# NorthStarUAS/ImageAnalysis

Measured on AMD Instinct MI355X. Metric: image_pairs_matched_per_sec, higher is better.
Workload: dtype u8 (int8 MFMA, int32 accumulate)

## Files before the change

imageanalysis_amd/csrc/match_knn2sym.hip:

```cpp
#include "iamx_common.h"
#include "sym_cand_rule.h"

namespace {

typedef int v4i __attribute__((ext_vector_type(4)));
typedef int v2i __attribute__((ext_vector_type(2)));
typedef int v16i __attribute__((ext_vector_type(16)));
typedef unsigned v2u __attribute__((ext_vector_type(2)));

#ifndef IAMX_DESC_OFFSET
#define IAMX_DESC_OFFSET 128
#endif
constexpr int D = IAMX_DESC_DIM;
constexpr int CHUNK = 128;
constexpr int BIG = 0x3F000000;

struct Pack3Args {
    const void *src;
    const int64_t *src_off;
    int64_t single_n;
    const int32_t *dst_off;
    int8_t *dst;
    int32_t *sn2, *sct, *sperm, *sinv;
    int32_t *n2, *nb, *pos;
// ... 183 lines not shown
            P.sn2[d0 + r] = 0;
            P.sct[d0 + r] = BIG;
            P.sperm[d0 + r] = -1;
            P.sinv[d0 + r] = -1;
        }
        return;
    }
    const SRC *p = static_cast<const SRC *>(P.src) + (r0 + r) * D + part * 16;
    unsigned w[4] = {0, 0, 0, 0};
#pragma unroll
    for (int i = 0; i < 16; ++i)
        w[i >> 2] |= (unsigned)((load_value(p, i) - IAMX_DESC_OFFSET) & 0xFF) << (8 * (i & 3));
    const int pos = d0 + P.pos[r0 + r];
    *reinterpret_cast<uint4 *>(P.dst + (int64_t)pos * D + part * 16) = make_uint4(w[0], w[1], w[2], w[3]);
    if (part == 0) {
        P.sn2[pos] = P.n2[r0 + r];
        P.sct[pos] = P.nb[r0 + r] >> 1;
        P.sperm[pos] = r;
        P.sinv[d0 + r] = pos - d0;
    }
}

constexpr int ROW_NO_BOUND = 0x7F000000;
__device__ __forceinline__ int pack_row_bounds(int L, int U1, int U2)
{
#if defined(IAMX_T_NOPACK)
    return U1;
#else
    typedef unsigned short us2 __attribute__((ext_vector_type(2)));
    const us2 d = __builtin_amdgcn_cvt_pk_u16((unsigned)(U1 - L), (unsigned)(U2 - L));
    return (int)__builtin_bit_cast(unsigned, d);
#endif
}
__device__ __forceinline__ void unpack_row_bounds(v2i e, int &L, int &U1, int &U2)
{
    const int d1 = e.y & 0xFFFF, d2 = (int)((unsigned)e.y >> 16);
    L = e.x;
    U1 = d1 == 0xFFFF ? ROW_NO_BOUND : e.x + d1;
    U2 = d2 == 0xFFFF ? ROW_NO_BOUND : e.x + d2;
}

struct SymArgs {
    const int8_t *sdesc;
    const int32_t *sn2, *sct;
    const int32_t *img_off, *img_n;
    const int32_t *upairs;
    const int32_t *wg_off;
    const int64_t *col_off;
    const int64_t *rowp_off;
    int32_t *col;
    int32_t *rowp;
    int n_u, total_wg;
    uint8_t *colmask;
};

__device__ __forceinline__ int uniform32(int x) { return __builtin_amdgcn_readfirstlane(x); }
__device__ __forceinline__ int64_t uniform64(int64_t x)
{
    return (int64_t)(((uint64_t)(unsigned)__builtin_amdgcn_readfirstlane((int)(x >> 32)) << 32) |
                     (unsigned)__builtin_amdgcn_readfirstlane((int)x));
}

template <bool FUSED>
__device__ __forceinline__ void half_wave_min16(int (&r)[16], int lo, int &m0, int &m1)
{
    int u[4], w[2];
    if constexpr (FUSED) {
        asm("s_nop 1\n\t"
            "v_min_i32_dpp %0, %0, %0 row_ror:8 row_mask:0xf bank_mask:0x3\n\t"
            "v_min_i32_dpp %0, %8, %8 row_ror:8 row_mask:0xf bank_mask:0xc\n\t"
            "v_min_i32_dpp %1, %1, %1 row_ror:8 row_mask:0xf bank_mask:0x3\n\t"
            "v_min_i32_dpp %1, %9, %9 row_ror:8 row_mask:0xf bank_mask:0xc\n\t"
            "v_min_i32_dpp %2, %2, %2 row_ror:8 row_mask:0xf bank_mask:0x3\n\t"
            "v_min_i32_dpp %2, %10, %10 row_ror:8 row_mask:0xf bank_mask:0xc\n\t"
            "v_min_i32_dpp %3, %3, %3 row_ror:8 row_mask:0xf bank_mask:0x3\n\t"
            "v_min_i32_dpp %3, %11, %11 row_ror:8 row_mask:0xf bank_mask:0xc\n\t"
            "v_min_i32_dpp %4, %4, %4 row_ror:8 row_mask:0xf bank_mask:0x3\n\t"
            "v_min_i32_dpp %4, %12, %12 row_ror:8 row_mask:0xf bank_mask:0xc\n\t"
            "v_min_i32_dpp %5, %5, %5 row_ror:8 row_mask:0xf bank_mask:0x3\n\t"
            "v_min_i32_dpp %5, %13, %13 row_ror:8 row_mask:0xf bank_mask:0xc\n\t"
            "v_min_i32_dpp %6, %6, %6 row_ror:8 row_mask:0xf bank_mask:0x3\n\t"
            "v_min_i32_dpp %6, %14, %14 row_ror:8 row_mask:0xf bank_mask:0xc\n\t"
            "v_min_i32_dpp %7, %7, %7 row_ror:8 row_mask:0xf bank_mask:0x3\n\t"
            "v_min_i32_dpp %7, %15, %15 row_ror:8 row_mask:0xf bank_mask:0xc"
            : "+v"(r[0]), "+v"(r[2]), "+v"(r[4]), "+v"(r[6]), "+v"(r[8]), "+v"(r[10]), "+v"(r[12]), "+v"(r[14])
            : "v"(r[1]), "v"(r[3]), "v"(r[5]), "v"(r[7]), "v"(r[9]), "v"(r[11]), "v"(r[13]), "v"(r[15]));
        asm("s_nop 1\n\t"
            "v_min_i32_dpp %0, %0, %0 row_ror:12 row_mask:0xf bank_mask:0x5\n\t"
            "v_min_i32_dpp %0, %4, %4 row_ror:4 row_mask:0xf bank_mask:0xa\n\t"
            "v_min_i32_dpp %1, %1, %1 row_ror:12 row_mask:0xf bank_mask:0x5\n\t"
            "v_min_i32_dpp %1, %5, %5 row_ror:4 row_mask:0xf bank_mask:0xa\n\t"
            "v_min_i32_dpp %2, %2, %2 row_ror:12 row_mask:0xf bank_mask:0x5\n\t"
            "v_min_i32_dpp %2, %6, %6 row_ror:4 row_mask:0xf bank_mask:0xa\n\t"
            "v_min_i32_dpp %3, %3, %3 row_ror:12 row_mask:0xf bank_mask:0x5\n\t"
            "v_min_i32_dpp %3, %7, %7 row_ror:4 row_mask:0xf bank_mask:0xa"
            : "+v"(r[0]), "+v"(r[4]), "+v"(r[8]), "+v"(r[12])
            : "v"(r[2]), "v"(r[6]), "v"(r[10]), "v"(r[14]));
#pragma unroll
        for (int k = 0; k < 4; ++k) u[k] = r[4 * k] + lo;
    } else {
        int s[8];
#pragma unroll
        for (int k = 0; k < 8; ++k) {
            const int a = r[2 * k], b = r[2 * k + 1];
            const int t1 = __builtin_amdgcn_update_dpp(b, a, 0x128, 0xF, 0x3, false);
            const int t2 = __builtin_amdgcn_update_dpp(a, b, 0x128, 0xF, 0xC, false);
// ... 55 lines not shown
            "v_min_i32_dpp %1, %1, %1 row_ror:12 row_mask:0xf bank_mask:0x5\n\t"
            "v_min_i32_dpp %1, %5, %5 row_ror:4 row_mask:0xf bank_mask:0xa\n\t"
            "v_min_i32_dpp %2, %2, %2 row_ror:12 row_mask:0xf bank_mask:0x5\n\t"
            "v_min_i32_dpp %2, %6, %6 row_ror:4 row_mask:0xf bank_mask:0xa\n\t"
            "v_min_i32_dpp %3, %3, %3 row_ror:12 row_mask:0xf bank_mask:0x5\n\t"
            "v_min_i32_dpp %3, %7, %7 row_ror:4 row_mask:0xf bank_mask:0xa"
            : "+v"(r[0]), "+v"(r[4]), "+v"(r[8]), "+v"(r[12])
            : "v"(r[2]), "v"(r[6]), "v"(r[10]), "v"(r[14]));
#pragma unroll
        for (int k = 0; k < 4; ++k) u[k] = r[4 * k] + lo;
    } else {
        int w[2];
#pragma unroll
        for (int k = 0; k < 2; ++k) {
            const v2u x = __builtin_amdgcn_permlane16_swap((unsigned)u[2 * k], (unsigned)u[2 * k + 1], false, false);
            w[k] = min((int)x[0], (int)x[1]);
        }
#pragma unroll
        for (int k = 0; k < 2; ++k) {
            w[k] = min(w[k], __builtin_amdgcn_update_dpp(0, w[k], 0xB1, 0xF, 0xF, true));
            w[k] = min(w[k], __builtin_amdgcn_update_dpp(0, w[k], 0x4E, 0xF, 0xF, true));
        }
        dst[0] = w[0];
        dst[16] = w[1];
    }
}

template <int P, bool PASS>
__device__ __forceinline__ void row_min16_block(int (&r)[16], int &after)
{
    static_assert(P >= 0 && P < 6, "six blocks");
    int keep = after;
    if constexpr (P < 4) {
        asm("s_nop 1\n\t"
            "v_min_i32_dpp %0, %0, %0 row_ror:8 row_mask:0xf bank_mask:0x3\n\t"
            "v_min_i32_dpp %0, %3, %3 row_ror:8 row_mask:0xf bank_mask:0xc\n\t"
            "v_min_i32_dpp %1, %1, %1 row_ror:8 row_mask:0xf bank_mask:0x3\n\t"
            "v_min_i32_dpp %1, %4, %4 row_ror:8 row_mask:0xf bank_mask:0xc"
            : "+v"(r[4 * P]), "+v"(r[4 * P + 2]), "+v"(keep)
            : "v"(r[4 * P + 1]), "v"(r[4 * P + 3]));
    } else {
        constexpr int Q = 8 * (P - 4);
        asm("s_nop 1\n\t"
            "v_min_i32_dpp %0, %0, %0 row_ror:12 row_mask:0xf bank_mask:0x5\n\t"
            "v_min_i32_dpp %0, %3, %3 row_ror:4 row_mask:0xf bank_mask:0xa\n\t"
            "v_min_i32_dpp %1, %1, %1 row_ror:12 row_mask:0xf bank_mask:0x5\n\t"
            "v_min_i32_dpp %1, %4, %4 row_ror:4 row_mask:0xf bank_mask:0xa"
            : "+v"(r[Q]), "+v"(r[Q + 4]), "+v"(keep)
            : "v"(r[Q + 2]), "v"(r[Q + 6]));
    }
    if constexpr (PASS) after = keep;
}

constexpr int sweep_gap_valu(int nv, int tail, bool blocks, int g)
{
    const int last = tail < 6 ? 6 - tail : 0;
    const int rest = nv - last - (blocks ? 2 : 0), n = blocks ? 5 : 7;
    if (g == 7) return last;
    if (blocks && (g == 3 || g == 4)) return 1;
    const int i = blocks && g > 4 ? g - 2 : g;
    return rest / n + (i < rest % n ? 1 : 0);
}

template <int V> struct int_c { static constexpr int value = V; };
template <int FROM, int TO, typename F>
__device__ __forceinline__ void static_for(F &&f)
{
    if constexpr (FROM < TO) {
        f(int_c<FROM>{});
        static_for<FROM + 1, TO>(f);
    }
}

template <int QW, int NW, int VARIANT, int PIPE, int MERGEW, int SLEEP, bool GROUPLO, int CH, int WPE>
__global__ __launch_bounds__(NW * 64, WPE) void knn2sym_kernel(SymArgs A)
{
    static_assert((VARIANT == 0 || VARIANT == 1) && PIPE > 0 && MERGEW == 2 && SLEEP == 0 && GROUPLO && CH == 128,
                  "only the shipped sweep is implemented");
    constexpr bool ITEMS = VARIANT == 1;
    constexpr int CHUNK = CH;
    constexpr int WGROWS = NW * QW * 32;
    constexpr int NT = NW * 64;
    constexpr int PIECES = CHUNK * D / 16 / NT;
    __shared__ __attribute__((aligned(16))) int8_t lds[2 * CHUNK * D + 2 * CHUNK * 4 + 3 * NW * CHUNK * 4 + 2 * NW * 4 + (2 * NW * CHUNK + NW * 256) * 4];
    int8_t *lds_tile = lds;
    int *lds_tb = reinterpret_cast<int *>(lds + 2 * CHUNK * D);
    int *lds_row = lds_tb + 2 * CHUNK;
    int *lds_cq = lds_row + 3 * NW * CHUNK;
    int *lds_dump = lds_cq + 2 * NW;
    const int tid = threadIdx.x, lane = tid & 63, wave = tid >> 6;
    const int c = lane & 31, g = lane >> 5;

    int vid;
    {
        const int total = A.total_wg, bid = blockIdx.x;
        const int xcd = bid & 7, k = bid >> 3, q = total >> 3, r = total & 7;
        vid = (xcd < r ? xcd * (q + 1) : r * (q + 1) + (xcd - r) * q) + k;
    }
    int lo = 0, hi = A.n_u;
    if constexpr (!ITEMS)
        while (hi - lo > 1) {
            const int mid = (lo + hi) >> 1;
            if (A.wg_off[mid] <= vid) lo = mid; else hi = mid;
        }
    int u = lo, u_end = 0, item_wgi = 0;
    if constexpr (ITEMS) {
        u = A.wg_off[3 * vid];
        u_end = u + A.wg_off[3 * vid + 1];
        item_wgi = A.wg_off[3 * vid + 2];
    }
    v4i bq[QW][4];
    int lo_lane;
    int bimg_held = -1;
    if constexpr (ITEMS) asm volatile("" : "+v"(u_end), "+v"(item_wgi), "+v"(bimg_held));
    int nx_b = 0, nx_a = 0, nx_boff = 0, nx_nb = 0, nx_aoff = 0, nx_na = 0;
    int64_t nx_rowp = 0;
    if constexpr (ITEMS) {
        nx_b = A.upairs[2 * u];
        nx_a = A.upairs[2 * u + 1];
        nx_boff = A.img_off[nx_b];
        nx_nb = A.img_n[nx_b];
        nx_aoff = A.img_off[nx_a];
        nx_na = A.img_n[nx_a];
        nx_rowp = A.rowp_off[u];
    }
    for (;;) {
        const int bimg = ITEMS ? uniform32(nx_b) : A.upairs[2 * u], aimg = ITEMS ? uniform32(nx_a) : A.upairs[2 * u + 1];
        const int boff = ITEMS ? uniform32(nx_boff) : A.img_off[bimg], nb = ITEMS ? uniform32(nx_nb) : A.img_n[bimg];
        const int aoff = ITEMS ? uniform32(nx_aoff) : A.img_off[aimg], na = ITEMS ? uniform32(nx_na) : A.img_n[aimg];
        const int capA = (na + CHUNK - 1) / CHUNK * CHUNK;
        const int nchunks = capA / CHUNK;
        const int wgi = ITEMS ? uniform32(item_wgi) : vid - A.wg_off[u];
        const int q0 = wgi * WGROWS + wave * (QW * 32);
        const bool wave_valid = q0 < nb;
        const int64_t rbase = (ITEMS ? uniform64(nx_rowp) : A.rowp_off[u]) + (int64_t)wgi * capA;
        if constexpr (ITEMS)
            if (uniform32(bimg_held) >= 0) __syncthreads();

        const int rc = (c & 16) | ((c & 3) << 2) | ((c >> 2) & 3);
        if (!ITEMS || bimg != uniform32(bimg_held)) {
            bimg_held = bimg;
#pragma unroll
            for (int qb = 0; qb < QW; ++qb) {
                int row = q0 + QW * rc + qb;
                row = row < nb ? row : nb - 1;
                const v4i *src = reinterpret_cast<const v4i *>(A.sdesc + (int64_t)(boff + row) * D);
#pragma unroll
                for (int s = 0; s < 4; ++s) {
                    bq[qb][s] = ~src[2 * s + g];
                    if constexpr (WPE == 1) asm volatile("" : "+a"(bq[qb][s]));
                }
            }
            lo_lane = 0;
            {
                int spread = 0;
                if (wave_valid) {
                    const int g_lo = rc & ~3, g_hi = rc | 3;
                    const int r_lo = q0 + QW * g_lo < nb ? q0 + QW * g_lo : nb - 1;
                    const int r_hi = q0 + QW * g_hi + QW - 1 < nb ? q0 + QW * g_hi + QW - 1 : nb - 1;
                    lo_lane = A.sn2[boff + r_lo] >> 1;
                    spread = (A.sn2[boff + r_hi] >> 1) - lo_lane;
                }
#pragma unroll
                for (int sh = 32; sh >= 1; sh >>= 1) spread = max(spread, __shfl_xor(spread, sh));
                if (lane == 0) lds_cq[wave] = spread;
            }
        }
// ... 14 lines not shown
        auto stage_direct = [&](int ch, int buf) {
#pragma unroll
            for (int j = 0; j < PIECES; ++j) {
                const int e = j * NT + tid, row = e >> 3, slot = (e & 7) ^ ((row >> 1) & 7);
                const int8_t *gsrc = tbase + (int64_t)(ch * CHUNK + row) * D + slot * 16;
                int8_t *ldst = lds_tile + buf * (CHUNK * D) + (j * NT + wave * 64) * 16;
                __builtin_amdgcn_global_load_lds(gsrc, (lds_ptr)ldst, 16, 0, 0);
            }
            __builtin_amdgcn_global_load_lds(tci + ch * CHUNK + (tid & (CHUNK - 1)),
                                             (lds_ptr)(lds_tb + buf * CHUNK + (wave & (CHUNK / 64 - 1)) * 64), 4, 0, 0);
        };
        auto wait_direct = [&]() { __builtin_amdgcn_s_waitcnt(0x0F70); };
        constexpr int MROWS = CHUNK / MERGEW;
        static_assert(MROWS == 64 && NW % MERGEW == 0, "one merge row per lane");
        const int mrow = (wave % MERGEW) * MROWS + lane;
        const bool merger = wave < MERGEW;
        constexpr int RSRC_WORD3_DATA_FORMAT_32 = 4 << 15;
        constexpr int RANGE_DROP = 0x7FFFFFF0;
        const __amdgpu_buffer_rsrc_t rowp_rsrc =
            __builtin_amdgcn_make_buffer_rsrc(A.rowp + 2 * rbase, (short)0, capA * 8, RSRC_WORD3_DATA_FORMAT_32);
        int spread_w[NW];
        auto merge_rows = [&](int ch, int rbo, bool store) {
            int L = BIG, U1 = BIG, U2 = BIG;
#pragma unroll
            for (int w = 0; w < NW; ++w) {
                const int R = lds_row[rbo + w * CHUNK + mrow];
                const int lw = R, uw = R + spread_w[w];
                L = min(L, lw);
                U2 = min(max(U1, uw), U2);
                U1 = min(U1, uw);
            }
            __builtin_amdgcn_raw_buffer_store_b64(v2i{L, pack_row_bounds(L, U1, U2)}, rowp_rsrc,
                                                  store ? (ch * CHUNK + mrow) * 8 : RANGE_DROP, 0, 0);
        };

        constexpr int PP = QW / 2, NT4 = CHUNK / 32, NS = NT4 * PP;
        static_assert(NT4 % 2 == 0 && NT4 >= 2, "tile parity must carry across chunks");
        int *const row_dst = (lane & 3) == 0 && wave_valid
            ? lds_row + wave * CHUNK + 8 * ((lane >> 4) & 1) + 4 * g + 2 * ((lane >> 2) & 1) + ((lane >> 3) & 1)
            : lds_dump + wave * 256 + lane;
        v4i aop[2][4], tbop[2][4];
        v16i accs[2][2];
        int r[2][16], bu[4];
#pragma unroll
        for (int k = 0; k < 16; ++k) r[1][k] = BIG;
        auto load_op = [&](int buf, int tile, int k, v4i (&a)[4], v4i (&tbv)[4]) {
            if (k < 4) {
                tbv[k] = *reinterpret_cast<const v4i *>(lds_tb + buf * CHUNK + tile * 32 + 8 * k + 4 * g);
            } else {
                const int s = k - 4, rr = tile * 32 + c, swz = (rr >> 1) & 7;
                a[s] = *reinterpret_cast<const v4i *>(lds_tile + buf * (CHUNK * D) + rr * D + (((2 * s + g) ^ swz) * 16));
            }
        };
        auto issue = [&](int t, int qp, v16i &acc0, v16i &acc1) {
#pragma unroll
            for (int reg = 0; reg < 16; ++reg) acc0[reg] = acc1[reg] = tbop[t & 1][reg >> 2][reg & 3];
#pragma unroll
            for (int s = 0; s < 4; ++s) {
                acc0 = __builtin_amdgcn_mfma_i32_32x32x32_i8(aop[t & 1][s], bq[qp][s], acc0, 0, 0, 0);
                acc1 = __builtin_amdgcn_mfma_i32_32x32x32_i8(aop[t & 1][s], bq[qp + 1][s], acc1, 0, 0, 0);
            }
            if constexpr (WPE == 1) asm volatile("" : "+v"(acc0), "+v"(acc1));
        };

        if constexpr (ITEMS) {
            const int un = u + 1 < u_end ? u + 1 : u;
            nx_b = A.upairs[2 * un];
            nx_a = A.upairs[2 * un + 1];
            nx_rowp = A.rowp_off[un];
        }
        stage_direct(0, 0);
        stage_direct(nchunks > 1 ? 1 : 0, 1);
        wait_direct();
        __syncthreads();
#pragma unroll
        for (int w = 0; w < NW; ++w) spread_w[w] = __builtin_amdgcn_readfirstlane(lds_cq[w]);
        if constexpr (ITEMS) {
            const int b = uniform32(nx_b), a = uniform32(nx_a);
            nx_boff = A.img_off[b];
            nx_nb = A.img_n[b];
            nx_aoff = A.img_off[a];
            nx_na = A.img_n[a];
        }
#pragma unroll
        for (int k = 0; k < 8; ++k) load_op(0, 0, k, aop[0], tbop[0]);
#pragma unroll
        for (int k = 0; k < 8 / PP; ++k) load_op(0, 1, k, aop[1], tbop[1]);
        issue(0, 0, accs[0][0], accs[0][1]);
        __builtin_amdgcn_sched_barrier(0);
        int rbo = 0, rbo_prev = 2 * NW * CHUNK;
        const int wave_u = uniform32(wave);
        typedef __attribute__((address_space(3))) const int8_t *lds_bytes;
        int opoff[4], tboff = 2 * CHUNK * D + 16 * g;
#pragma unroll
        for (int s = 0; s < 4; ++s) opoff[s] = c * D + (((2 * s + g) ^ ((c >> 1) & 7)) * 16);
        auto load_op_at = [&](int tile, int k, v4i (&a)[4], v4i (&tbv)[4]) {
            if (k < 4) tbv[k] = *reinterpret_cast<const __attribute__((address_space(3))) v4i *>((lds_bytes)lds + tboff + tile * 128 + 32 * k);
            else a[k - 4] = *reinterpret_cast<const __attribute__((address_space(3))) v4i *>((lds_bytes)lds + opoff[k - 4] + tile * (32 * D));
        };
        const unsigned stage_voff = (unsigned)((tid >> 3) * D + (((tid & 7) ^ ((tid >> 4) & 7)) * 16));
        const unsigned ct_voff = (unsigned)((tid & (CHUNK - 1)) * 4);
        for (int ch = 0; ch < nchunks; ++ch) {
            const int buf = ch & 1;
            if constexpr (PP == 4) {
            constexpr int BAR = (NT4 - 1) * PP - 1;
            static_assert(NW == 4 && PIECES == 4 && BAR + 4 < NS && (NT / 8) % 16 == 0, "the gaps below are form 2's");
            const int chs = ch + 2 < nchunks ? ch + 2 : nchunks - 1;
            const int8_t *const sg_tile = tbase + (int64_t)chs * (CHUNK * D);
            const int8_t *const sg_ct = reinterpret_cast<const int8_t *>(tci + chs * CHUNK);
            int mR[NW], mL = BIG, mU1 = BIG, mU2 = BIG;
            static_for<0, NS>([&](auto st_c) {
                constexpr int st = decltype(st_c)::value;
                constexpr int t = st / PP, ph = st % PP, qp = 2 * ph, cur = st & 1;
                constexpr int nst = st + 1 < NS ? st + 1 : 0;
                if constexpr (st == BAR) {
                    __builtin_amdgcn_s_waitcnt(0x0070);
                    __syncthreads();
                }
                issue(nst / PP, 2 * (nst % PP), accs[cur ^ 1][0], accs[cur ^ 1][1]);
                static_for<(st == BAR - 1 ? 1 : 0), (st == BAR - 2 ? 2 : 1)>([&](auto d_c) {
                    constexpr int sr = st + decltype(d_c)::value;
                    constexpr int T = (sr + 1) / PP + 1, i = (sr + 1) % PP;
                    if constexpr (T == NT4 && i == 0) {
#pragma unroll
                        for (int s = 0; s < 4; ++s) opoff[s] ^= CHUNK * D;
                        tboff ^= CHUNK * 4;
                    }
#pragma unroll
                    for (int k = i * 8 / PP; k < (i + 1) * 8 / PP; ++k) load_op_at(T % NT4, k, aop[T & 1], tbop[T & 1]);
                });
                constexpr int nv = (ph == 2 ? 36 : ph == 3 ? 40 : 32) + (st == BAR + 2 ? 11 : 0) + (st == BAR + 3 ? 5 : 0) +
                                   (st >= BAR && st <= BAR + PIECES ? 1 : 0) +
                                   (st == NS - 1 ? 2 : 0);
                constexpr int tail = (st == BAR - 1 ? 0 : st == BAR - 2 ? 4 : 2) + (ph == 3 ? 1 + 2 : 0) + (st >= BAR && st <= BAR + PIECES ? 1 : 0) +
                                     (st == BAR + 1 ? 2 : 0) + (st == BAR + 3 ? 1 : 0);
                constexpr int blk_at = sweep_gap_valu(nv, tail, true, 0) + sweep_gap_valu(nv, tail, true, 1) +
                                       sweep_gap_valu(nv, tail, true, 2) - 16;
                static_assert(ph == 3 || (blk_at >= 0 && blk_at < 15 && blk_at != 7), "gaps 3 and 4 hold two minima of one column chain");
                const v16i acc0 = accs[cur][0], acc1 = accs[cur][1];
                int (&rc_)[16] = r[t & 1];
                int (&rp)[16] = r[(t + 1) & 1];
#pragma unroll
                for (int reg = 0; reg < 16; ++reg)
                    rc_[reg] = qp == 0 ? min(acc0[reg], acc1[reg]) : min(min(rc_[reg], acc0[reg]), acc1[reg]);
                static_for<0, 16>([&](auto w_c) {
                    constexpr int w = decltype(w_c)::value;
                    int &mm = m[qp + (w >> 3)][t & 3];
                    const v16i &acc = w < 8 ? acc0 : acc1;
                    mm = min(min(mm, acc[2 * (w & 7)]), acc[2 * (w & 7) + 1]);
                    if constexpr (ph < 3 && w == blk_at) row_min16_block<2 * ph, true>(rp, mm);
                    if constexpr (ph < 3 && w == blk_at + 1) row_min16_block<2 * ph + 1, true>(rp, mm);
                });
                if constexpr (ph == 2) {
#pragma unroll
                    for (int k = 0; k < 4; ++k) bu[k] = rp[4 * k] + lo_lane;
                }
                if constexpr (ph == 3) {
                    int *const dst = row_dst + (t > 0 ? rbo : rbo_prev) + (t > 0 ? t - 1 : NT4 - 1) * 32;
                    row_min16_piece<3>(rp, bu, lo_lane, dst);
                }
                if constexpr (st >= BAR && st < BAR + PIECES)
                    __builtin_amdgcn_global_load_lds(sg_tile + (st - BAR) * ((NT / 8) * D) + stage_voff,
                                                     (lds_ptr)(lds_tile + buf * (CHUNK * D) + ((st - BAR) * NT + wave_u * 64) * 16), 16, 0, 0);
                if constexpr (st == BAR + PIECES)
                    __builtin_amdgcn_global_load_lds(sg_ct + ct_voff,
                                                     (lds_ptr)(lds_tb + buf * CHUNK + (wave_u & (CHUNK / 64 - 1)) * 64), 4, 0, 0);
                if constexpr (st == BAR + 1) {
#pragma unroll
                    for (int w = 0; w < NW; ++w) mR[w] = lds_row[rbo_prev + w * CHUNK + mrow];
                }
                if constexpr (st == BAR + 2) {
#pragma unroll
                    for (int w = 0; w < NW; ++w) {
                        const int uw = mR[w] + spread_w[w];
                        mL = min(mL, mR[w]);
                        mU2 = min(max(mU1, uw), mU2);
                        mU1 = min(mU1, uw);
                    }
                }
                if constexpr (st == BAR + 3)
                    __builtin_amdgcn_raw_buffer_store_b64(v2i{mL, pack_row_bounds(mL, mU1, mU2)}, rowp_rsrc,
                                                          merger && ch > 0 ? ((ch - 1) * CHUNK + mrow) * 8 : RANGE_DROP, 0, 0);
                static_for<0, 8>([&](auto g_c) {
                    constexpr int g = decltype(g_c)::value;
                    __builtin_amdgcn_sched_group_barrier(0x008, 1, 0);
                    __builtin_amdgcn_sched_group_barrier(0x002, sweep_gap_valu(nv, tail, ph < 3, g) + (g == 7 ? 3 : 0), 0);
                });
                __builtin_amdgcn_sched_barrier(0);
            });
            } else {
#pragma unroll
            for (int st = 0; st < NS; ++st) {
                const int t = st / PP, qp = 2 * (st % PP), cur = st & 1;
                if (st == (NT4 - 1) * PP - 1) {
                    __builtin_amdgcn_s_waitcnt(0x0070);
                    __syncthreads();
                    stage_direct(ch + 2 < nchunks ? ch + 2 : nchunks - 1, buf);
                    merge_rows(ch - 1, rbo_prev, merger && ch > 0);
                }
                if (st + 1 < NS) issue((st + 1) / PP, 2 * ((st + 1) % PP), accs[cur ^ 1][0], accs[cur ^ 1][1]);
                else issue(0, 0, accs[cur ^ 1][0], accs[cur ^ 1][1]);
                {
                    const int T = (st + 1) / PP + 1, i = (st + 1) % PP;
#pragma unroll
                    for (int k = i * 8 / PP; k < (i + 1) * 8 / PP; ++k)
                        load_op(T < NT4 ? buf : buf ^ 1, T % NT4, k, aop[T & 1], tbop[T & 1]);
                }
                const v16i acc0 = accs[cur][0], acc1 = accs[cur][1];
                int t0 = min(min(m[qp][t & 3], acc0[0]), acc0[1]);
                int t1m = min(min(m[qp + 1][t & 3], acc1[0]), acc1[1]);
#pragma unroll
                for (int reg = 2; reg < 16; reg += 2) {
                    t0 = min(min(t0, acc0[reg]), acc0[reg + 1]);
                    t1m = min(min(t1m, acc1[reg]), acc1[reg + 1]);
                }
                m[qp][t & 3] = t0;
                m[qp + 1][t & 3] = t1m;
                int (&rc_)[16] = r[t & 1];
                if (qp == 0) {
#pragma unroll
                    for (int reg = 0; reg < 16; ++reg) rc_[reg] = min(acc0[reg], acc1[reg]);
                } else {
#pragma unroll
                    for (int reg = 0; reg < 16; ++reg) rc_[reg] = min(min(rc_[reg], acc0[reg]), acc1[reg]);
                }
                {
                    int (&rp)[16] = r[(t + 1) & 1];
                    const int tp = t > 0 ? t - 1 : NT4 - 1;
                    int *dst = row_dst + (t > 0 ? rbo : rbo_prev) + tp * 32;
                    if constexpr (PP == 1) {
                        int m0, m1;
                        half_wave_min16<true>(rp, lo_lane, m0, m1);
                        dst[0] = m0;
                        dst[16] = m1;
                    } else {
                        if (0 * PP / 4 == st % PP) row_min16_piece<0>(rp, bu, lo_lane, dst);
                        if (1 * PP / 4 == st % PP) row_min16_piece<1>(rp, bu, lo_lane, dst);
                        if (2 * PP / 4 == st % PP) row_min16_piece<2>(rp, bu, lo_lane, dst);
                        if (3 * PP / 4 == st % PP) row_min16_piece<3>(rp, bu, lo_lane, dst);
                    }
                }
#pragma unroll
                for (int i = 0; i < 8; ++i) {
                    __builtin_amdgcn_sched_group_barrier(0x008, 1, 0);
                    __builtin_amdgcn_sched_group_barrier(0x002, PIPE, 0);
                }
                __builtin_amdgcn_sched_barrier(0);
            }
            }
            rbo_prev = rbo;
            rbo = rbo == 2 * NW * CHUNK ? 0 : rbo + NW * CHUNK;
        }
        int64_t col_v = 0;
        if constexpr (ITEMS) col_v = A.col_off[u];
        {
            int m0, m1;
            half_wave_min16<true>(r[(NT4 - 1) & 1], lo_lane, m0, m1);
            int *dst = row_dst + rbo_prev + (NT4 - 1) * 32;
            dst[0] = m0;
            dst[16] = m1;
        }
        wait_direct();
        __syncthreads();
        merge_rows(nchunks - 1, rbo_prev, merger);

        const int64_t col_u = ITEMS ? uniform64(col_v) : 0;
        if (wave_valid) {
            unsigned ownpack = 0;
            int v1s[QW], v2s[QW];
#pragma unroll
            for (int qb = 0; qb < QW; ++qb) {
                const int lo01 = min(m[qb][0], m[qb][1]), hi01 = max(m[qb][0], m[qb][1]);
                const int lo23 = min(m[qb][2], m[qb][3]), hi23 = max(m[qb][2], m[qb][3]);
                const int a1 = min(lo01, lo23), a2 = min(max(lo01, lo23), min(hi01, hi23));
                const int b1 = __shfl_xor(a1, 32), b2 = __shfl_xor(a2, 32);
                const int v1 = min(a1, b1), v2 = min(max(a1, b1), min(a2, b2));
                v1s[qb] = v1;
                v2s[qb] = v2;
#if !defined(IAMX_T_NOMASK)
                const unsigned own = (m[qb][0] <= v2 ? 1u : 0u) | (m[qb][1] <= v2 ? 2u : 0u) |
                                     (m[qb][2] <= v2 ? 4u : 0u) | (m[qb][3] <= v2 ? 8u : 0u);
                ownpack |= own << (4 * qb);
#endif
            }
            const unsigned othpack = A.colmask ? (unsigned)__shfl_xor((int)ownpack, 32) : 0u;
            const int row0 = q0 + QW * rc;
            if (g == 0) {
#pragma unroll
                for (int qb = 0; qb < QW; ++qb)
                    if (row0 + qb < nb)
                        *reinterpret_cast<v2i *>(A.col + 2 * ((ITEMS ? col_u : A.col_off[u]) + row0 + qb)) = v2i{v1s[qb], v2s[qb]};
                if (A.colmask) {
                    uint8_t *dst = A.colmask + (ITEMS ? col_u : A.col_off[u]) + row0;
                    if (QW == 8 && row0 + QW <= nb) {
                        auto spread = [](unsigned nib4) {
                            const unsigned x = (nib4 | (nib4 << 8)) & 0x00FF00FFu;
                            return (x | (x << 4)) & 0x0F0F0F0Fu;
                        };
                        const unsigned lo = spread(ownpack & 0xFFFFu) | (spread(othpack & 0xFFFFu) << 4);
                        const unsigned hi = spread(ownpack >> 16) | (spread(othpack >> 16) << 4);
                        *reinterpret_cast<v2u *>(dst) = v2u{lo, hi};
                    } else {
#pragma unroll
                        for (int qb = 0; qb < QW; ++qb)
                            if (row0 + qb < nb)
// ... 1055 lines not shown
                       dim3((unsigned)(((int64_t)cap * 8 + 255) / 256), (unsigned)P.n_img),
                       dim3(256), 0, st, P);
    return iamx::check_launch(what);
}

template <typename SRC>
static int pack3_single(const SRC *src, int64_t n_rows, int8_t *dst, int32_t *sn2, int32_t *sct,
                        int32_t *sperm, int32_t *sinv, int32_t *scratch, void *stream,
                        const char *what)
{
    if (n_rows < 0 || n_rows > (1 << 24) || (n_rows > 0 && !src) || !dst || !sn2 || !sct || !sperm ||
        !sinv || !scratch)
        return iamx::fail(IAMX_EINVAL, "%s: null pointer or bad row count", what);
    Pack3Args P{src, nullptr, n_rows, nullptr, dst, sn2, sct, sperm, sinv,
                scratch, scratch + n_rows, scratch + 2 * n_rows, 1};
    return pack3_launch<SRC>(P, n_rows, (int)n_rows, stream, what);
}

extern "C" int iamx_desc3_pack_u8(const uint8_t *src, int64_t n_rows, int8_t *dst, int32_t *sn2,
                                  int32_t *sct, int32_t *sperm, int32_t *sinv, int32_t *scratch,
                                  void *stream)
{
    return pack3_single(src, n_rows, dst, sn2, sct, sperm, sinv, scratch, stream, "iamx_desc3_pack_u8");
}

extern "C" int iamx_desc3_pack_f32(const float *src, int64_t n_rows, int8_t *dst, int32_t *sn2,
                                   int32_t *sct, int32_t *sperm, int32_t *sinv, int32_t *scratch,
                                   void *stream)
{
    return pack3_single(src, n_rows, dst, sn2, sct, sperm, sinv, scratch, stream, "iamx_desc3_pack_f32");
}

extern "C" int iamx_desc3_pack_batch_u8(const uint8_t *src, const int64_t *src_off,
                                        const int32_t *dst_off, int n_img, int64_t total_rows,
                                        int max_rows_per_image, int8_t *dst, int32_t *sn2,
                                        int32_t *sct, int32_t *sperm, int32_t *sinv,
                                        int32_t *scratch, void *stream)
{
    IAMX_REQUIRE(src && src_off && dst_off && dst && sn2 && sct && sperm && sinv && scratch,
                 "null pointer");
    IAMX_REQUIRE(n_img > 0 && total_rows >= 0 && max_rows_per_image >= 0, "bad count");
    Pack3Args P{src, src_off, 0, dst_off, dst, sn2, sct, sperm, sinv,
                scratch, scratch + total_rows, scratch + 2 * total_rows, n_img};
    return pack3_launch<uint8_t>(P, total_rows, max_rows_per_image, stream, "iamx_desc3_pack_batch_u8");
}

#define SWEEP_FORM2 8, 4, 0, 5, 2, 0, true, 128, 1
#define SWEEP_FORM1 4, 4, 0, 6, 2, 0, true, 128, 2
#define SWEEP_FORM0 2, 4, 0, 6, 2, 0, true, 128, 2
#define SWEEP_ITEMS2 8, 4, 1, 5, 2, 0, true, 128, 1
#define SWEEP_STR2(...) #__VA_ARGS__
#define SWEEP_STR(...) SWEEP_STR2(__VA_ARGS__)

extern "C" const char *iamx_knn2sym_kernel_id(int form)
{
    switch (form) {
    case 2: return "knn2sym_kernel<" SWEEP_STR(SWEEP_ITEMS2) ">";
    case 1: return "knn2sym_kernel<" SWEEP_STR(SWEEP_FORM1) ">";
    case 0: return "knn2sym_kernel<" SWEEP_STR(SWEEP_FORM0) ">";
    default: return "";
    }
}

extern "C" int iamx_knn2sym_sweep(const int8_t *sdesc, const int32_t *sn2, const int32_t *sct,
                                  const int32_t *img_off, const int32_t *img_n,
                                  const int32_t *upairs, const int32_t *wg_off,
                                  const int64_t *col_off, const int64_t *rowp_off, int n_u,
                                  int total_wg, int form, int32_t *col, int32_t *rowp,
                                  uint8_t *colmask, void *stream)
{
    IAMX_REQUIRE(sdesc && sn2 && sct && img_off && img_n && upairs && wg_off && col_off && rowp_off &&
                     col && rowp,
                 "null pointer");
    IAMX_REQUIRE(n_u >= 0 && total_wg >= 0, "negative count");
    IAMX_REQUIRE(form >= 0 && form <= 2, "form must be 0 (256 rows), 1 (512) or 2 (1024)");
    if (n_u == 0 || total_wg == 0) return IAMX_OK;
    SymArgs a{sdesc, sn2, sct, img_off, img_n, upairs, wg_off, col_off, rowp_off, col, rowp, n_u, total_wg,
              colmask};
    const dim3 g((unsigned)total_wg);
    hipStream_t st = iamx::as_stream(stream);
    if (form == 2) hipLaunchKernelGGL((knn2sym_kernel<SWEEP_FORM2>), g, dim3(256), 0, st, a);
    else if (form == 1) hipLaunchKernelGGL((knn2sym_kernel<SWEEP_FORM1>), g, dim3(256), 0, st, a);
    else hipLaunchKernelGGL((knn2sym_kernel<SWEEP_FORM0>), g, dim3(256), 0, st, a);
    return iamx::check_launch("iamx_knn2sym_sweep");
}

extern "C" int iamx_knn2sym_sweep_items(const int8_t *sdesc, const int32_t *sn2, const int32_t *sct,
                                        const int32_t *img_off, const int32_t *img_n,
                                        const int32_t *upairs, const int32_t *items,
                                        const int64_t *col_off, const int64_t *rowp_off, int n_u,
                                        int n_items, int32_t *col, int32_t *rowp, uint8_t *colmask,
                                        void *stream)
{
    IAMX_REQUIRE(sdesc && sn2 && sct && img_off && img_n && upairs && items && col_off && rowp_off &&
                     col && rowp,
                 "null pointer");
    IAMX_REQUIRE(n_u >= 0 && n_items >= 0, "negative count");
    if (n_u == 0 || n_items == 0) return IAMX_OK;
    SymArgs a{sdesc, sn2, sct, img_off, img_n, upairs, items, col_off, rowp_off, col, rowp, n_u, n_items,
              colmask};
    hipLaunchKernelGGL((knn2sym_kernel<SWEEP_ITEMS2>), dim3((unsigned)n_items), dim3(256), 0,
                       iamx::as_stream(stream), a);
    return iamx::check_launch("iamx_knn2sym_sweep_items");
}

static bool narrow_enabled()
{
    const char *e = getenv("IAMX_EXACT_NARROW");
    return !(e && e[0] == '0');
}

extern "C" int64_t iamx_knn2sym_narrow_bytes(int64_t rows, int n_pairs)
{
    if (rows <= 0 || n_pairs <= 0) return 0;
    return narrow_layout(rows, n_pairs).total;
}

extern "C" int iamx_knn2sym_candidates(const int32_t *sn2, const int32_t *sperm,
                                       const int32_t *img_off, const int32_t *img_n,
                                       const int32_t *pairs, const int32_t *osrc,
                                       const int32_t *wg_off, const int64_t *col_off,
                                       const int64_t *rowp_off, const int64_t *out_off,
                                       const int32_t *col, const int32_t *rowp, int n_pairs,
                                       double thresh, uint8_t *keep, int32_t *cand_cnt,
                                       int32_t *cand_q, int32_t *task_total, int32_t *tasks,
                                       int32_t *d2, const uint8_t *colmask, void *nar,
                                       int64_t rows_total, int max_query_rows, int form, void *stream)
{
    IAMX_REQUIRE(sn2 && sperm && img_off && img_n && pairs && osrc && wg_off && col_off && rowp_off &&
                     out_off && col && rowp && keep && cand_cnt && cand_q && task_total && tasks && d2,
                 "null pointer");
    IAMX_REQUIRE(!nar || colmask, "narrow workspace without colmask");
    IAMX_REQUIRE(form >= 0 && form <= 2, "form must be 0, 1 or 2");
    if (n_pairs <= 0) return IAMX_OK;
    CandArgs a{sn2, sperm, img_off, img_n, pairs, osrc, wg_off, col_off, rowp_off, out_off, col, rowp,
               thresh, sym_cand_K(thresh), keep, cand_cnt, cand_q, task_total, tasks, d2, 8,
               colmask, narrow_enabled() ? static_cast<int8_t *>(nar) : nullptr, rows_total, n_pairs,
               iamx_knn2sym_rows_per_wg(form)};
    IAMX_REQUIRE(rows_total > 0 && rows_total < (1ll << 31), "rows_total = rows of all ordered pairs");
    IAMX_REQUIRE(max_query_rows > 0, "max_query_rows = rows of the largest query image");
    const int64_t keep_words = (rows_total + 31) / 32;
    const int64_t clear_wg = (keep_words + 4095) / 4096;
    hipLaunchKernelGGL(symcand_clear_kernel, dim3((unsigned)(clear_wg < 256 ? clear_wg : 256)), dim3(256), 0,
                       iamx::as_stream(stream), reinterpret_cast<unsigned *>(keep), keep_words, cand_cnt, n_pairs);
    hipLaunchKernelGGL(symcand_rows_kernel,
                       dim3((unsigned)((max_query_rows + 1023) / 1024), (unsigned)(n_pairs < 65535 ? n_pairs : 65535)),
                       dim3(256), 0, iamx::as_stream(stream), a);
    hipLaunchKernelGGL(symcand_kernel, dim3((unsigned)n_pairs), dim3(256), 0, iamx::as_stream(stream), a);
    return iamx::check_launch("iamx_knn2sym_candidates");
}

extern "C" int iamx_knn2sym_exact(const int8_t *desc, const int32_t *norm_q, const int32_t *norm_t,
                                  int32_t *key_t, int64_t total_rows,
// ... 45 lines not shown
```

Measured before the change: 624,400.

## Interleave LDS staging loads and min reductions inside the MFMA sweep schedule

Replaces the compiler global_load_lds builtins with inline-asm staging that sets m0 and is placed at a fixed slot inside the column-min chain. The row and column min updates are reordered into one interleaved 32-step sequence, and the scheduling gaps are adjusted to match. Operand LDS reads and the accumulator pinning now come after the reductions, and the double-buffer offset flip moves to the barrier stage. Also adds compile-time-gated s_memtime instrumentation, which is off by default. The aim is to hide global-to-LDS staging and VALU min work under the MFMA stream, at the cost of fragile hand scheduling and m0 save/restore overhead.

```diff
diff --git a/imageanalysis_amd/csrc/match_knn2sym.hip b/imageanalysis_amd/csrc/match_knn2sym.hip
--- a/imageanalysis_amd/csrc/match_knn2sym.hip
+++ b/imageanalysis_amd/csrc/match_knn2sym.hip
@@ -259,6 +259,9 @@
     int32_t *rowp;
     int n_u, total_wg;
     uint8_t *colmask;
+#if defined(IAMX_T_STAMPS)
+    unsigned long long *stamps;
+#endif
 };
 
 __device__ __forceinline__ int uniform32(int x) { return __builtin_amdgcn_readfirstlane(x); }
@@ -420,6 +423,30 @@
     if constexpr (PASS) after = keep;
 }
 
+template <int BYTES>
+__device__ __forceinline__ void stage_piece_held(const void *gsrc, unsigned lds_dst, int &after)
+{
+    static_assert(BYTES == 16 || BYTES == 4, "one dwordx4 or one dword a lane");
+    unsigned m0_was;
+    int keep = after;
+    if constexpr (BYTES == 16)
+        asm volatile("s_mov_b32 %0, m0\n\ts_mov_b32 m0, %3\n\ts_nop 0\n\tglobal_load_lds_dwordx4 %2, off\n\ts_mov_b32 m0, %0"
+                     : "=&s"(m0_was), "+v"(keep) : "v"(gsrc), "s"(lds_dst) : "memory");
+    else
+        asm volatile("s_mov_b32 %0, m0\n\ts_mov_b32 m0, %3\n\ts_nop 0\n\tglobal_load_lds_dword %2, off\n\ts_mov_b32 m0, %0"
+                     : "=&s"(m0_was), "+v"(keep) : "v"(gsrc), "s"(lds_dst) : "memory");
+    after = keep;
+}
+
+#if defined(IAMX_T_STAMPS)
+#define SWEEP_STAMP(t)                                                                     \
+    do {                                                                                   \
+        __builtin_amdgcn_sched_barrier(0);                                                 \
+        asm volatile("s_memtime %0\n\ts_waitcnt lgkmcnt(0)" : "=s"(t) : : "memory");       \
+        __builtin_amdgcn_sched_barrier(0);                                                 \
+    } while (0)
+#endif
+
 constexpr int sweep_gap_valu(int nv, int tail, bool blocks, int g)
 {
     const int last = tail < 6 ? 6 - tail : 0;
@@ -428,6 +455,15 @@
     if (blocks && (g == 3 || g == 4)) return 1;
     const int i = blocks && g > 4 ? g - 2 : g;
     return rest / n + (i < rest % n ? 1 : 0);
+}
+
+constexpr int sweep_min_order(bool blocks, int p3, int i)
+{
+    const int head = blocks ? 6 : 8;
+    if (i < head) return 16 + i;
+    if (blocks && (i == p3 || i == p3 + 1)) return 16 + 6 + (i - p3);
+    const int f = i - (blocks && i < p3 ? 6 : 8);
+    return f < 8 ? 24 + f : f - 8;
 }
 
 template <int V> struct int_c { static constexpr int value = V; };
@@ -481,6 +517,9 @@
     int lo_lane;
     int bimg_held = -1;
     if constexpr (ITEMS) asm volatile("" : "+v"(u_end), "+v"(item_wgi), "+v"(bimg_held));
+#if defined(IAMX_T_STAMPS)
+    unsigned long long stamp_sum = 0, stamp_chunks = 0, stamp_cycles = 0, stamp_ticks = 0;
+#endif
     int nx_b = 0, nx_a = 0, nx_boff = 0, nx_nb = 0, nx_aoff = 0, nx_na = 0;
     int64_t nx_rowp = 0;
     if constexpr (ITEMS) {
@@ -601,7 +640,10 @@
                 a[s] = *reinterpret_cast<const v4i *>(lds_tile + buf * (CHUNK * D) + rr * D + (((2 * s + g) ^ swz) * 16));
             }
         };
-        auto issue = [&](int t, int qp, v16i &acc0, v16i &acc1) {
+        auto pin_accs = [&](v16i &acc0, v16i &acc1) {
+            if constexpr (WPE == 1) asm volatile("" : "+v"(acc0), "+v"(acc1));
+        };
+        auto issue = [&](int t, int qp, v16i &acc0, v16i &acc1, bool pin = true) {
 #pragma unroll
             for (int reg = 0; reg < 16; ++reg) acc0[reg] = acc1[reg] = tbop[t & 1][reg >> 2][reg & 3];
 #pragma unroll
@@ -609,7 +651,7 @@
                 acc0 = __builtin_amdgcn_mfma_i32_32x32x32_i8(aop[t & 1][s], bq[qp][s], acc0, 0, 0, 0);
                 acc1 = __builtin_amdgcn_mfma_i32_32x32x32_i8(aop[t & 1][s], bq[qp + 1][s], acc1, 0, 0, 0);
             }
-            if constexpr (WPE == 1) asm volatile("" : "+v"(acc0), "+v"(acc1));
+            if (pin) pin_accs(acc0, acc1);
         };
 
         if constexpr (ITEMS) {
@@ -648,7 +690,13 @@
             else a[k - 4] = *reinterpret_cast<const __attribute__((address_space(3))) v4i *>((lds_bytes)lds + opoff[k - 4] + tile * (32 * D));
         };
         const unsigned stage_voff = (unsigned)((tid >> 3) * D + (((tid & 7) ^ ((tid >> 4) & 7)) * 16));
+        const unsigned lds_tile_at = (unsigned)(uintptr_t)(lds_ptr)(lds_tile + wave_u * (64 * 16));
+        const unsigned lds_tb_at = (unsigned)(uintptr_t)(lds_ptr)(lds_tb + (wave_u & (CHUNK / 64 - 1)) * 64);
         const unsigned ct_voff = (unsigned)((tid & (CHUNK - 1)) * 4);
+#if defined(IAMX_T_STAMPS)
+        const unsigned long long loop_c0 = __builtin_amdgcn_s_memtime(), loop_r0 = __builtin_amdgcn_s_memrealtime();
+        __builtin_amdgcn_s_waitcnt(0xC07F);
+#endif
         for (int ch = 0; ch < nchunks; ++ch) {
             const int buf = ch & 1;
             if constexpr (PP == 4) {
@@ -662,44 +710,81 @@
                 constexpr int st = decltype(st_c)::value;
                 constexpr int t = st / PP, ph = st % PP, qp = 2 * ph, cur = st & 1;
                 constexpr int nst = st + 1 < NS ? st + 1 : 0;
+#if defined(IAMX_T_STAMPS)
+                unsigned long long stamp_t0 = 0, stamp_t1 = 0;
+                if constexpr (IAMX_T_STAMPS == st + 1 || (st == BAR && IAMX_T_STAMPS == 17)) SWEEP_STAMP(stamp_t0);
+                if constexpr (st == 0 && IAMX_T_STAMPS == 19) {
+                    SWEEP_STAMP(stamp_t0);
+                    SWEEP_STAMP(stamp_t1);
+                    stamp_sum += stamp_t1 - stamp_t0;
+                }
+#endif
                 if constexpr (st == BAR) {
                     __builtin_amdgcn_s_waitcnt(0x0070);
+#if defined(IAMX_T_STAMPS)
+                    if constexpr (IAMX_T_STAMPS == 17) {
+                        SWEEP_STAMP(stamp_t1);
+                        stamp_sum += stamp_t1 - stamp_t0;
+                    }
+                    if constexpr (IAMX_T_STAMPS == 18) SWEEP_STAMP(stamp_t0);
+#endif
                     __syncthreads();
-                }
-                issue(nst / PP, 2 * (nst % PP), accs[cur ^ 1][0], accs[cur ^ 1][1]);
-                static_for<(st == BAR - 1 ? 1 : 0), (st == BAR - 2 ? 2 : 1)>([&](auto d_c) {
-                    constexpr int sr = st + decltype(d_c)::value;
-                    constexpr int T = (sr + 1) / PP + 1, i = (sr + 1) % PP;
-                    if constexpr (T == NT4 && i == 0) {
-#pragma unroll
-                        for (int s = 0; s < 4; ++s) opoff[s] ^= CHUNK * D;
-                        tboff ^= CHUNK * 4;
+#if defined(IAMX_T_STAMPS)
+                    if constexpr (IAMX_T_STAMPS == 18) {
+                        SWEEP_STAMP(stamp_t1);
+                        stamp_sum += stamp_t1 - stamp_t0;
                     }
-#pragma unroll
-                    for (int k = i * 8 / PP; k < (i + 1) * 8 / PP; ++k) load_op_at(T % NT4, k, aop[T & 1], tbop[T & 1]);
-                });
+#endif
+                }
+                issue(nst / PP, 2 * (nst % PP), accs[cur ^ 1][0], accs[cur ^ 1][1], false);
+                auto operand_reads = [&]() {
+                    static_for<(st == BAR - 1 ? 1 : 0), (st == BAR - 2 ? 2 : 1)>([&](auto d_c) {
+                        constexpr int sr = st + decltype(d_c)::value;
+                        constexpr int T = (sr + 1) / PP + 1, i = (sr + 1) % PP;
+#pragma unroll
+                        for (int k = i * 8 / PP; k < (i + 1) * 8 / PP; ++k) load_op_at(T % NT4, k, aop[T & 1], tbop[T & 1]);
+                    });
+                };
+                if constexpr (st == BAR) {
+#pragma unroll
+                    for (int s = 0; s < 4; ++s) opoff[s] ^= CHUNK * D;
+                    tboff ^= CHUNK * 4;
+                }
                 constexpr int nv = (ph == 2 ? 36 : ph == 3 ? 40 : 32) + (st == BAR + 2 ? 11 : 0) + (st == BAR + 3 ? 5 : 0) +
                                    (st >= BAR && st <= BAR + PIECES ? 1 : 0) +
                                    (st == NS - 1 ? 2 : 0);
-                constexpr int tail = (st == BAR - 1 ? 0 : st == BAR - 2 ? 4 : 2) + (ph == 3 ? 1 + 2 : 0) + (st >= BAR && st <= BAR + PIECES ? 1 : 0) +
+                constexpr int tail = (st == BAR - 1 ? 0 : st == BAR - 2 ? 4 : 2) + (ph == 3 ? 1 + 2 : 0) +
                                      (st == BAR + 1 ? 2 : 0) + (st == BAR + 3 ? 1 : 0);
+                constexpr bool staging = st >= BAR && st <= BAR + PIECES;
+                constexpr int STAGE_GAP = 1, STAGE_AT = 8 + 1;
                 constexpr int blk_at = sweep_gap_valu(nv, tail, true, 0) + sweep_gap_valu(nv, tail, true, 1) +
-                                       sweep_gap_valu(nv, tail, true, 2) - 16;
-                static_assert(ph == 3 || (blk_at >= 0 && blk_at < 15 && blk_at != 7), "gaps 3 and 4 hold two minima of one column chain");
+                                       sweep_gap_valu(nv, tail, true, 2) - (staging ? 2 : 0);
+                static_assert(ph == 3 || (blk_at >= 6 && blk_at < 31), "gaps 3 and 4 hold the last two minima of column chain 0");
                 const v16i acc0 = accs[cur][0], acc1 = accs[cur][1];
                 int (&rc_)[16] = r[t & 1];
                 int (&rp)[16] = r[(t + 1) & 1];
-#pragma unroll
-                for (int reg = 0; reg < 16; ++reg)
-                    rc_[reg] = qp == 0 ? min(acc0[reg], acc1[reg]) : min(min(rc_[reg], acc0[reg]), acc1[reg]);
-                static_for<0, 16>([&](auto w_c) {
-                    constexpr int w = decltype(w_c)::value;
-                    int &mm = m[qp + (w >> 3)][t & 3];
-                    const v16i &acc = w < 8 ? acc0 : acc1;
-                    mm = min(min(mm, acc[2 * (w & 7)]), acc[2 * (w & 7) + 1]);
-                    if constexpr (ph < 3 && w == blk_at) row_min16_block<2 * ph, true>(rp, mm);
-                    if constexpr (ph < 3 && w == blk_at + 1) row_min16_block<2 * ph + 1, true>(rp, mm);
+                static_for<0, 32>([&](auto i_c) {
+                    constexpr int i = decltype(i_c)::value, op = sweep_min_order(ph < 3, blk_at, i);
+                    if constexpr (op < 16) {
+                        rc_[op] = qp == 0 ? min(acc0[op], acc1[op]) : min(min(rc_[op], acc0[op]), acc1[op]);
+                    } else {
+                        constexpr int w = op - 16;
+                        int &mm = m[qp + (w >> 3)][t & 3];
+                        const v16i &acc = w < 8 ? acc0 : acc1;
+                        mm = min(min(mm, acc[2 * (w & 7)]), acc[2 * (w & 7) + 1]);
+                        if constexpr (ph < 3 && i == blk_at) row_min16_block<2 * ph, true>(rp, mm);
+                        if constexpr (ph < 3 && i == blk_at + 1) row_min16_block<2 * ph + 1, true>(rp, mm);
+                        if constexpr (staging && w == STAGE_AT) {
+                            if constexpr (st < BAR + PIECES)
+                                stage_piece_held<16>(sg_tile + (st - BAR) * ((NT / 8) * D) + stage_voff,
+                                                     lds_tile_at + buf * (CHUNK * D) + (st - BAR) * NT * 16, mm);
+                            else
+                                stage_piece_held<4>(sg_ct + ct_voff, lds_tb_at + buf * (CHUNK * 4), mm);
+                        }
+                    }
                 });
+                pin_accs(accs[cur ^ 1][0], accs[cur ^ 1][1]);
+                operand_reads();
                 if constexpr (ph == 2) {
 #pragma unroll
                     for (int k = 0; k < 4; ++k) bu[k] = rp[4 * k] + lo_lane;
@@ -708,12 +793,6 @@
                     int *const dst = row_dst + (t > 0 ? rbo : rbo_prev) + (t > 0 ? t - 1 : NT4 - 1) * 32;
                     row_min16_piece<3>(rp, bu, lo_lane, dst);
                 }
-                if constexpr (st >= BAR && st < BAR + PIECES)
-                    __builtin_amdgcn_global_load_lds(sg_tile + (st - BAR) * ((NT / 8) * D) + stage_voff,
-                                                     (lds_ptr)(lds_tile + buf * (CHUNK * D) + ((st - BAR) * NT + wave_u * 64) * 16), 16, 0, 0);
-                if constexpr (st == BAR + PIECES)
-                    __builtin_amdgcn_global_load_lds(sg_ct + ct_voff,
-                                                     (lds_ptr)(lds_tb + buf * CHUNK + (wave_u & (CHUNK / 64 - 1)) * 64), 4, 0, 0);
                 if constexpr (st == BAR + 1) {
 #pragma unroll
                     for (int w = 0; w < NW; ++w) mR[w] = lds_row[rbo_prev + w * CHUNK + mrow];
@@ -733,9 +812,16 @@
                 static_for<0, 8>([&](auto g_c) {
                     constexpr int g = decltype(g_c)::value;
                     __builtin_amdgcn_sched_group_barrier(0x008, 1, 0);
-                    __builtin_amdgcn_sched_group_barrier(0x002, sweep_gap_valu(nv, tail, ph < 3, g) + (g == 7 ? 3 : 0), 0);
+                    __builtin_amdgcn_sched_group_barrier(0x002, sweep_gap_valu(nv, tail, ph < 3, g) + (g == 7 ? 3 : 0) -
+                                                                    (staging && g == STAGE_GAP ? 1 : 0), 0);
                 });
                 __builtin_amdgcn_sched_barrier(0);
+#if defined(IAMX_T_STAMPS)
+                if constexpr (IAMX_T_STAMPS == st + 1) {
+                    SWEEP_STAMP(stamp_t1);
+                    stamp_sum += stamp_t1 - stamp_t0;
+                }
+#endif
             });
             } else {
 #pragma unroll
@@ -800,6 +886,22 @@
             rbo_prev = rbo;
             rbo = rbo == 2 * NW * CHUNK ? 0 : rbo + NW * CHUNK;
         }
+#if defined(IAMX_T_STAMPS)
+        if constexpr (PP == 4) {
+            unsigned long long loop_c1;
+            SWEEP_STAMP(loop_c1);
+            stamp_cycles += loop_c1 - loop_c0;
+            stamp_ticks += __builtin_amdgcn_s_memrealtime() - loop_r0;
+            stamp_chunks += (unsigned)nchunks;
+            if (A.stamps && lane == 0) {
+                unsigned long long *o = A.stamps + ((size_t)blockIdx.x * NW + wave) * 4;
+                o[0] = stamp_sum;
+                o[1] = stamp_chunks;
+                o[2] = stamp_cycles;
+                o[3] = stamp_ticks;
+            }
+        }
+#endif
         int64_t col_v = 0;
         if constexpr (ITEMS) col_v = A.col_off[u];
         {
@@ -1961,6 +2063,18 @@
 #define SWEEP_STR2(...) #__VA_ARGS__
 #define SWEEP_STR(...) SWEEP_STR2(__VA_ARGS__)
 
+#if defined(IAMX_T_STAMPS)
+static unsigned long long *g_sweep_stamps = nullptr;
+extern "C" int iamx_knn2sym_set_stamps(void *buf)
+{
+    g_sweep_stamps = static_cast<unsigned long long *>(buf);
+    return IAMX_OK;
+}
+#define SWEEP_STAMPS_ARG , g_sweep_stamps
+#else
+#define SWEEP_STAMPS_ARG
+#endif
+
 extern "C" const char *iamx_knn2sym_kernel_id(int form)
 {
     switch (form) {
@@ -1985,7 +2099,7 @@
     IAMX_REQUIRE(form >= 0 && form <= 2, "form must be 0 (256 rows), 1 (512) or 2 (1024)");
     if (n_u == 0 || total_wg == 0) return IAMX_OK;
     SymArgs a{sdesc, sn2, sct, img_off, img_n, upairs, wg_off, col_off, rowp_off, col, rowp, n_u, total_wg,
-              colmask};
+              colmask SWEEP_STAMPS_ARG};
     const dim3 g((unsigned)total_wg);
     hipStream_t st = iamx::as_stream(stream);
     if (form == 2) hipLaunchKernelGGL((knn2sym_kernel<SWEEP_FORM2>), g, dim3(256), 0, st, a);
@@ -2007,7 +2121,7 @@
     IAMX_REQUIRE(n_u >= 0 && n_items >= 0, "negative count");
     if (n_u == 0 || n_items == 0) return IAMX_OK;
     SymArgs a{sdesc, sn2, sct, img_off, img_n, upairs, items, col_off, rowp_off, col, rowp, n_u, n_items,
-              colmask};
+              colmask SWEEP_STAMPS_ARG};
     hipLaunchKernelGGL((knn2sym_kernel<SWEEP_ITEMS2>), dim3((unsigned)n_items), dim3(256), 0,
                        iamx::as_stream(stream), a);
     return iamx::check_launch("iamx_knn2sym_sweep_items");
```

Result: faster. 633,000 (median of 6 runs) (+1.4%).
